# matsengrp/linearham

Hardware: AMD Instinct MI355X
Metric: phylo-HMM log-likelihood evals/sec (100-leaf x 400-site family) (higher is better)
Workload: dtype f64

## Files before the change

### linearham_amd/csrc/lh_forward.hip

```cpp
#include <cstdio>
#include <cstdlib>
#include <type_traits>

#include "lh_device.h"

namespace lh {

constexpr int kFwdThreads = 256;
constexpr int kFwdWaves = kFwdThreads / 64;
constexpr int kJunctionWaves = 4;

thread_local char g_k2a_form[64] = "", g_k2b_form[32] = "", g_forward_form[160] = "";
thread_local int g_k2b_dj_samples = 0;
thread_local int g_k2b_dj_waves = 0;

__device__ static inline int block_max_int(int v, int* red, int phase) {
#pragma unroll
  for (int off = 32; off > 0; off >>= 1) v = max(v, __shfl_xor(v, off, 64));
  int* r = red + phase * kFwdWaves;
  if ((threadIdx.x & 63) == 0) r[threadIdx.x >> 6] = v;
  __syncthreads();
  return max(max(r[0], r[1]), max(r[2], r[3]));
}

// ... 473 lines not shown
      lem[j] = l;
    }
  }
  if constexpr (kExt) {
    const int W1 = fam.vd.n_rows, W2 = fam.has_d ? fam.dj.n_rows : 0, NP = fam.n_prune;
    int32_t* jrs = jrs_all + s * (size_t)(W1 + W2);
    for (int r = tid; r < W1 + W2; r += kFwdThreads) {
      const int pat = r < W1 ? fam.vd.row_pat[r] : fam.dj.row_pat[r - W1];
      int smin = 0;
      if (kFromSiteLik && pat < NP) {
        smin = 0x7fffffff;
        for (int q = 0; q < R; ++q) smin = min(smin, site_scal[(s * R + q) * NP + pat]);
      }
      jrs[r] = smin;
    }
  }

  const int nV = fam.vgerm.n_genes, nD = fam.dgerm.n_genes, nJ = fam.jgerm.n_genes;
  double* gem = gem_all + s * fam.gem_size;
  const bool direct = *em_bad != 0;
  auto fill = [&](const DevSegments& seg, double* out, int phase) {
    if constexpr (kExt) return fill_segments_ext<kG, kByteOff>(seg, em, ems, tid, out, redi, phase);
    if (seg.cons_sites > 0 && !direct)
      return fill_consensus<kG, kByteOff>(seg, em, tid, out, redi, phase, cons_inv, cons_pv, cons_pk, cons_cap);
    return fill_segments<kG, kByteOff>(seg, em, tid, out, redi, phase);
  };
  int cv = fill(fam.vpadding, gem, 0);
  cv += fill(fam.vgerm, gem + nV, 1);
  int cd = 0, cj;
  if (small_sets_by_wave(fam, kExt, direct)) {
    const int wave = tid >> 6, lane = tid & 63;
    double* jg = gem + 2 * (size_t)nV + (fam.has_d ? nD : 0);
    int m = 0;
    if (wave == 1 && fam.has_d) m = fill_segments_wave<kByteOff>(fam.dgerm, em, lane, gem + 2 * (size_t)nV);
    if (wave == 2) m = fill_segments_wave<kByteOff>(fam.jgerm, em, lane, jg);
    if (wave == 3) m = fill_segments_wave<kByteOff>(fam.jpadding, em, lane, jg + nJ);
    if (lane == 0) redi[wave] = m;
    __syncthreads();
    cd = redi[1];
    cj = redi[2] + redi[3];
  } else if (fam.has_d) {
    cd = fill(fam.dgerm, gem + 2 * (size_t)nV, 0);
    cj = fill(fam.jgerm, gem + 2 * (size_t)nV + nD, 1);
    cj += fill(fam.jpadding, gem + 2 * (size_t)nV + nD + nJ, 0);
  } else {
    cj = fill(fam.jgerm, gem + 2 * (size_t)nV, 0);
    cj += fill(fam.jpadding, gem + 2 * (size_t)nV + nJ, 1);
  }
  if (tid == 0) {
    gcnt_all[s * 3 + 0] = cv;
    gcnt_all[s * 3 + 1] = cd;
    gcnt_all[s * 3 + 2] = cj;
  }
}


template <int kCtrl>
__device__ static inline double dpp_move(double v) {
  const int lo = __builtin_amdgcn_update_dpp(0, __double2loint(v), kCtrl, 0xf, 0xf, true);
  const int hi = __builtin_amdgcn_update_dpp(0, __double2hiint(v), kCtrl, 0xf, 0xf, true);
  return __hiloint2double(hi, lo);
}

__device__ static inline double read_lane(double v, int lane) {
  return __hiloint2double(__builtin_amdgcn_readlane(__double2hiint(v), lane),
                          __builtin_amdgcn_readlane(__double2loint(v), lane));
}

constexpr int kDppQuadSwap1 = 0xB1;
constexpr int kDppQuadSwap2 = 0x4E;
constexpr int kDppHalfMirror = 0x141;
constexpr int kDppMirror = 0x140;

__device__ static inline double wave_sum(double v) {
  v += dpp_move<kDppQuadSwap1>(v);
  v += dpp_move<kDppQuadSwap2>(v);
  v += dpp_move<kDppHalfMirror>(v);
  v += dpp_move<kDppMirror>(v);
  return (read_lane(v, 0) + read_lane(v, 16)) + (read_lane(v, 32) + read_lane(v, 48));
}

__device__ static inline unsigned scale_key(double v) { return (unsigned)__double2hiint(v) - 1u; }

template <int kCtrl>
__device__ static inline unsigned dpp_min_u32(unsigned v) {
  return min(v, (unsigned)__builtin_amdgcn_update_dpp(0, (int)v, kCtrl, 0xf, 0xf, true));
}

__device__ static inline unsigned wave_min_key(unsigned v) {
  v = dpp_min_u32<kDppQuadSwap1>(v);
  v = dpp_min_u32<kDppQuadSwap2>(v);
  v = dpp_min_u32<kDppHalfMirror>(v);
  v = dpp_min_u32<kDppMirror>(v);
  const unsigned a = __builtin_amdgcn_readlane((int)v, 0), b = __builtin_amdgcn_readlane((int)v, 16);
  const unsigned c = __builtin_amdgcn_readlane((int)v, 32), d = __builtin_amdgcn_readlane((int)v, 48);
  return min(min(a, b), min(c, d));
}

template <int kCtrl>
__device__ static inline unsigned dpp_max_u32(unsigned v) {
  return max(v, (unsigned)__builtin_amdgcn_update_dpp(0, (int)v, kCtrl, 0xf, 0xf, true));
}

__device__ static inline unsigned wave_max_u32(unsigned v) {
  v = dpp_max_u32<kDppQuadSwap1>(v);
  v = dpp_max_u32<kDppQuadSwap2>(v);
  v = dpp_max_u32<kDppHalfMirror>(v);
  v = dpp_max_u32<kDppMirror>(v);
  const unsigned a = __builtin_amdgcn_readlane((int)v, 0), b = __builtin_amdgcn_readlane((int)v, 16);
  const unsigned c = __builtin_amdgcn_readlane((int)v, 32), d = __builtin_amdgcn_readlane((int)v, 48);
  return max(max(a, b), max(c, d));
}

template <bool kExt>
__device__ static inline unsigned key_start() {
  return kExt ? 0u : 0xffffffffu;
}
template <bool kExt>
__device__ static inline unsigned key_add(unsigned key, double v) {
  return kExt ? max(key, (unsigned)__double2hiint(v)) : min(key, scale_key(v));
}

struct RowScale {
  int k;
  double factor;
  bool extra;
  __device__ double apply(double v) const {
    v *= factor;
    if (extra) v *= kScaleFactor;
    return v;
  }
};

__device__ static inline RowScale row_scale(unsigned min_key) {
  const unsigned hw = min_key + 1u;
  const unsigned e = (hw >> 20) & 0x7ffu;
  RowScale s;
  s.extra = hw != 0 && e == 0 && (hw & 0xfffffu) < (1u << 18);
  const int k3 = hw == 0 ? 0 : (e < 767u) + (e < 511u) + (e < 255u);
  s.k = k3 + (s.extra ? 1 : 0);
  s.factor = __hiloint2double((1023 + 256 * k3) << 20, 0);
  return s;
}

template <bool kExt>
__device__ static inline RowScale wave_row_scale(unsigned key) {
  return row_scale(kExt ? wave_max_u32(key) - 1u : wave_min_key(key));
}

__device__ static __forceinline__ RowScale pick(bool hi, const RowScale& sa, const RowScale& sb) {
  return RowScale{hi ? sb.k : sa.k, hi ? sb.factor : sa.factor, hi ? sb.extra : sa.extra};
}

struct RightRow {
  double nlo[4], rtr, rli;
  int ridx;
  int4 nx;
};

template <int GL, int GR>
struct RowTables {
  double ltr[GL], llo[GL];
  int lidx[GL];
  RightRow right[GR];
};

__device__ static __forceinline__ void load_right_row(const DevJunction& J, int i, unsigned r, RightRow& t) {
  const size_t orr = (size_t)i * J.right_pad;
  const double2* pn = reinterpret_cast<const double2*>(J.right_nlo) + 2 * orr;
  const double2 a = pn[2u * r], b = pn[2u * r + 1u];
  t.nlo[0] = a.x;
  t.nlo[1] = a.y;
  t.nlo[2] = b.x;
  t.nlo[3] = b.y;
  t.nx = (reinterpret_cast<const int4*>(J.nti_xmsa) + orr)[r];
  t.rtr = (J.right_trans + orr)[r];
  t.rli = (J.right_gp_li + orr)[r];
  t.ridx = (J.right_xmsa + orr)[r];
}

template <int GL, int GR>
__device__ static inline void load_row(const DevJunction& J, int i, unsigned lane, RowTables<GL, GR>& t) {
  const size_t ol = (size_t)i * J.left_pad;
  const double* lt = J.left_trans + ol;
  const double* ll = J.left_lo + ol;
  const int32_t* lx = J.left_xmsa + ol;
#pragma unroll
  for (int q = 0; q < GL; ++q) {
    t.ltr[q] = lt[lane + 64u * q];
    t.llo[q] = ll[lane + 64u * q];
    t.lidx[q] = lx[lane + 64u * q];
  }
#pragma unroll
  for (int q = 0; q < GR; ++q) load_right_row(J, i, lane + 64u * q, t.right[q]);
}


__device__ static __forceinline__ void load_nli(const DevJunction& J, unsigned r, double (&nli)[4]) {
  const double2* p = reinterpret_cast<const double2*>(J.right_gp_nli) + 2u * r;
  const double2 a = p[0], b = p[1];
  nli[0] = a.x, nli[1] = a.y, nli[2] = b.x, nli[3] = b.y;
}

template <bool kExt>
__device__ static __forceinline__ unsigned right_gene_step(unsigned key, double (&fN)[4], double& fR, double A,
                                                           const double (&nli)[4], const double* ntt_lds, unsigned r,
                                                           const RightRow& t, const double* jem) {
  const double n0 = fN[0], n1 = fN[1], n2 = fN[2], n3 = fN[3];
  const double2* tt = reinterpret_cast<const double2*>(ntt_lds) + 8u * r;
  const int nxs[4] = {t.nx.x, t.nx.y, t.nx.z, t.nx.w};
#pragma unroll
  for (int b = 0; b < 4; ++b) {
    const double2 t01 = tt[2 * b], t23 = tt[2 * b + 1];
    double s = ((n0 * t01.x + n1 * t01.y) + n2 * t23.x) + n3 * t23.y;
    s += A * nli[b];
    fN[b] = s * jem[nxs[b]];
  }
  double s = ((n0 * t.nlo[0] + n1 * t.nlo[1]) + n2 * t.nlo[2]) + n3 * t.nlo[3];
  s += fR * t.rtr;
  s += A * t.rli;
  fR = s * jem[t.ridx];
#pragma unroll
  for (int b = 0; b < 4; ++b) key = key_add<kExt>(key, fN[b]);
  return key_add<kExt>(key, fR);
}

__device__ static __forceinline__ double exit_handoff(const DevJunction& J, unsigned r, int nR, const double (&fN)[4],
                                                      double fR, double A, const double* __restrict__ germ_em,
                                                      const double* __restrict__ pad_trans,
                                                      const double* __restrict__ pad_em) {
  const double2* xn = reinterpret_cast<const double2*>(J.exit_nlo) + 2u * r;
  const double2 x01 = xn[0], x23 = xn[1];
  double s = ((fN[0] * x01.x + fN[1] * x01.y) + fN[2] * x23.x) + fN[3] * x23.y;
  s += fR * J.exit_trans[r];
  s += A * J.exit_gp_li[r];
  double v = 0.0;
  if ((int)r < nR) {
    v = s * germ_em[r];
    if (pad_trans) v *= pad_trans[r];
    if (pad_em) v *= pad_em[r];
  }
  return v;
}

__device__ static __forceinline__ void store_right(double* __restrict__ o, int nL, int nR, unsigned r,
                                                   const double (&fN)[4], double fR) {
  if ((int)r < nR) {
    o[nL + 4 * (size_t)r + 0] = fN[0];
    o[nL + 4 * (size_t)r + 1] = fN[1];
    o[nL + 4 * (size_t)r + 2] = fN[2];
    o[nL + 4 * (size_t)r + 3] = fN[3];
    o[nL + 4 * (size_t)nR + r] = fR;
  }
}

__device__ static __forceinline__ size_t junction_fwd_size(const DevJunction& J) {
  return (size_t)J.n_rows * (J.n_left + 5 * (size_t)J.n_right);
}

template <int GL, int GR, bool kExt>
__device__ static int junction_wave(const DevJunction& J, const double* jem, const double* ntt_lds, int lane,
                                    const double (&f_in)[GL], int count_in, const double* __restrict__ germ_em,
                                    const double* __restrict__ pad_trans, const double* __restrict__ pad_em,
                                    double (&g_out)[GR], double* __restrict__ fwd_out,
                                    int32_t* __restrict__ scal_out, const int32_t* __restrict__ jrs) {
  const int W = J.n_rows, nL = J.n_left, nR = J.n_right;
  int count = count_in;
  double fL[GL], fN[GR][4], fR[GR];
  double nli[GR][4];
#pragma unroll
  for (int q = 0; q < GL; ++q) fL[q] = f_in[q];
#pragma unroll
  for (int q = 0; q < GR; ++q) {
    fR[q] = 0.0;
    fN[q][0] = fN[q][1] = fN[q][2] = fN[q][3] = 0.0;
    load_nli(J, lane + 64u * q, nli[q]);
  }
  const size_t row_stride = (size_t)nL + 5 * (size_t)nR;
  double A;
  {
    double part = 0.0;
#pragma unroll
    for (int q = 0; q < GL; ++q) part += f_in[q] * J.enter_lo[lane + 64u * q];
    A = wave_sum(part);
  }

  auto step = [&](int i, const RowTables<GL, GR>& t) __attribute__((always_inline)) {
    unsigned key = key_start<kExt>();
    double part = 0.0;
#pragma unroll
    for (int q = 0; q < GL; ++q) {
      const double v = (fL[q] * t.ltr[q]) * jem[t.lidx[q]];
      fL[q] = v;
      key = key_add<kExt>(key, v);
      part += v * t.llo[q];
    }
#pragma unroll
    for (int q = 0; q < GR; ++q)
      key = right_gene_step<kExt>(key, fN[q], fR[q], A, nli[q], ntt_lds, lane + 64u * q, t.right[q], jem);
    A = wave_sum(part);
    const RowScale sc = wave_row_scale<kExt>(key);
    if constexpr (kExt) count += jrs[i];
    if (sc.k != 0) {
      A = sc.apply(A);
#pragma unroll
      for (int q = 0; q < GL; ++q) fL[q] = sc.apply(fL[q]);
#pragma unroll
      for (int q = 0; q < GR; ++q) {
        fR[q] = sc.apply(fR[q]);
#pragma unroll
        for (int b = 0; b < 4; ++b) fN[q][b] = sc.apply(fN[q][b]);
      }
      count += sc.k;
    }
    if (fwd_out) {
      double* o = fwd_out + (size_t)i * row_stride;
#pragma unroll
      for (int q = 0; q < GL; ++q) {
        const int g = lane + 64 * q;
        if (g < nL) o[g] = fL[q];
      }
#pragma unroll
      for (int q = 0; q < GR; ++q) store_right(o, nL, nR, lane + 64u * q, fN[q], fR[q]);
    }
    if (scal_out && lane == 0) scal_out[i] = count;
  };

  for (int i = 0; i < W; ++i) {
    RowTables<GL, GR> t;
    load_row<GL, GR>(J, i, lane, t);
    step(i, t);
  }

  unsigned key = key_start<kExt>();
#pragma unroll
  for (int q = 0; q < GR; ++q) {
    const double v = exit_handoff(J, lane + 64u * q, nR, fN[q], fR[q], A, germ_em, pad_trans, pad_em);
    key = key_add<kExt>(key, v);
    g_out[q] = v;
  }
  const RowScale last = wave_row_scale<kExt>(key);
#pragma unroll
  for (int q = 0; q < GR; ++q) g_out[q] = last.apply(g_out[q]);
  return count + last.k;
}


struct HalfPair {
  double a, b;
};

__device__ static inline HalfPair half_sums(double v) {
  v += dpp_move<kDppQuadSwap1>(v);
  v += dpp_move<kDppQuadSwap2>(v);
  v += dpp_move<kDppHalfMirror>(v);
  v += dpp_move<kDppMirror>(v);
  return HalfPair{read_lane(v, 0) + read_lane(v, 16), read_lane(v, 32) + read_lane(v, 48)};
}

struct HalfKeys {
  unsigned a, b;
};

template <bool kExt>
__device__ static inline HalfKeys half_keys(unsigned v) {
  if (kExt) {
    v = dpp_max_u32<kDppQuadSwap1>(v);
    v = dpp_max_u32<kDppQuadSwap2>(v);
    v = dpp_max_u32<kDppHalfMirror>(v);
    v = dpp_max_u32<kDppMirror>(v);
  } else {
    v = dpp_min_u32<kDppQuadSwap1>(v);
    v = dpp_min_u32<kDppQuadSwap2>(v);
    v = dpp_min_u32<kDppHalfMirror>(v);
    v = dpp_min_u32<kDppMirror>(v);
  }
  const unsigned a = __builtin_amdgcn_readlane((int)v, 0), b = __builtin_amdgcn_readlane((int)v, 16);
  const unsigned c = __builtin_amdgcn_readlane((int)v, 32), d = __builtin_amdgcn_readlane((int)v, 48);
  return kExt ? HalfKeys{max(a, b) - 1u, max(c, d) - 1u} : HalfKeys{min(a, b), min(c, d)};
}

template <bool kExt>
__device__ static int junction_pair(const DevJunction& J, const double* jem, const double* ntt_lds, int lane, bool hi,
                                    double f_in, int count_in, const double* __restrict__ germ_em,
                                    const double* __restrict__ pad_trans, const double* __restrict__ pad_em,
                                    double& g_out, double* __restrict__ fwd_out, int32_t* __restrict__ scal_out,
                                    const int32_t* __restrict__ jrs, bool valid) {
  const int W = J.n_rows, nL = J.n_left, nR = J.n_right;
  const unsigned g = lane & 31;
  int count = count_in;
  double fL = f_in, fR = 0.0, fN[4] = {0.0, 0.0, 0.0, 0.0}, nli[4];
  load_nli(J, g, nli);
  const size_t row_stride = (size_t)nL + 5 * (size_t)nR;
  auto mine = [&](const HalfPair& p) { return hi ? p.b : p.a; };
  double A = mine(half_sums(f_in * J.enter_lo[g]));
  for (int i = 0; i < W; ++i) {
    const size_t ol = (size_t)i * J.left_pad;
    const double ltr = J.left_trans[ol + g], llo = J.left_lo[ol + g];
    const int lidx = J.left_xmsa[ol + g];
    RightRow t;
    load_right_row(J, i, g, t);

    unsigned key = key_start<kExt>();
    {
      const double v = (fL * ltr) * jem[lidx];
      fL = v;
      key = key_add<kExt>(key, v);
    }
    const double part = fL * llo;
    key = right_gene_step<kExt>(key, fN, fR, A, nli, ntt_lds, g, t, jem);
    A = mine(half_sums(part));
    const HalfKeys hk = half_keys<kExt>(key);
    const RowScale sa = row_scale(hk.a), sb = row_scale(hk.b);
    if constexpr (kExt) count += jrs[i];
    if ((sa.k | sb.k) != 0) {
      const RowScale sc = pick(hi, sa, sb);
      A = sc.apply(A);
      fL = sc.apply(fL);
      fR = sc.apply(fR);
#pragma unroll
      for (int b = 0; b < 4; ++b) fN[b] = sc.apply(fN[b]);
      count += sc.k;
    }
    if (fwd_out && valid) {
      double* o = fwd_out + (size_t)i * row_stride;
      if ((int)g < nL) o[g] = fL;
      store_right(o, nL, nR, g, fN, fR);
    }
    if (scal_out && valid && g == 0) scal_out[i] = count;
  }
  g_out = exit_handoff(J, g, nR, fN, fR, A, germ_em, pad_trans, pad_em);
  const HalfKeys hk = half_keys<kExt>(key_add<kExt>(key_start<kExt>(), g_out));
  const RowScale last = pick(hi, row_scale(hk.a), row_scale(hk.b));
  g_out = last.apply(g_out);
  return count + last.k;
}

template <int GL, bool kExt>
__device__ static void junction_vd_pair(const DevJunction& J, const double* jemA, const double* jemB,
                                        const double* ntt_lds, int lane, bool hi, const double (&fA_in)[GL],
                                        const double (&fB_in)[GL], int countA_in, int countB_in,
                                        const double* __restrict__ germ_em_mine, double& g_out, int& count_mine,
                                        double* __restrict__ fwdA, double* __restrict__ fwdB,
                                        int32_t* __restrict__ scoA, int32_t* __restrict__ scoB,
                                        const int32_t* __restrict__ jrsA, const int32_t* __restrict__ jrsB) {
  const int W = J.n_rows, nL = J.n_left, nR = J.n_right;
  const unsigned g = lane & 31;
  const double* jemM = hi ? jemB : jemA;
  int countA = countA_in, countB = countB_in;
  double fA[GL], fB[GL], fN[4] = {0.0, 0.0, 0.0, 0.0}, fR = 0.0, nli[4];
#pragma unroll
  for (int q = 0; q < GL; ++q) {
    fA[q] = fA_in[q];
    fB[q] = fB_in[q];
  }
  load_nli(J, g, nli);
  const size_t row_stride = (size_t)nL + 5 * (size_t)nR;
  double AA, AB;
  {
    double pa = 0.0, pb = 0.0;
#pragma unroll
    for (int q = 0; q < GL; ++q) {
      const double lo = J.enter_lo[lane + 64u * q];
      pa += fA_in[q] * lo;
      pb += fB_in[q] * lo;
    }
    AA = wave_sum(pa);
    AB = wave_sum(pb);
  }
  auto combine = [](unsigned a, unsigned b) { return kExt ? max(a, b) : min(a, b); };
  for (int i = 0; i < W; ++i) {
    const size_t ol = (size_t)i * J.left_pad;
    unsigned keyA = key_start<kExt>(), keyB = key_start<kExt>();
    double partA = 0.0, partB = 0.0;
    {
      const double* lt = J.left_trans + ol;
      const double* ll = J.left_lo + ol;
      const int32_t* lx = J.left_xmsa + ol;
#pragma unroll
      for (int q = 0; q < GL; ++q) {
        const double ltr = lt[lane + 64u * q], llo = ll[lane + 64u * q];
        const int lidx = lx[lane + 64u * q];
        const double va = (fA[q] * ltr) * jemA[lidx];
        const double vb = (fB[q] * ltr) * jemB[lidx];
        fA[q] = va;
        fB[q] = vb;
        keyA = key_add<kExt>(keyA, va);
        keyB = key_add<kExt>(keyB, vb);
        partA += va * llo;
        partB += vb * llo;
      }
    }
    {
      RightRow t;
      load_right_row(J, i, g, t);
      const unsigned keyR = right_gene_step<kExt>(key_start<kExt>(), fN, fR, hi ? AB : AA, nli, ntt_lds, g, t, jemM);
      if (hi)
        keyB = combine(keyB, keyR);
      else
        keyA = combine(keyA, keyR);
    }
    AA = wave_sum(partA);
    AB = wave_sum(partB);
    const RowScale sa = wave_row_scale<kExt>(keyA), sb = wave_row_scale<kExt>(keyB);
    if constexpr (kExt) {
      countA += jrsA[i];
      countB += jrsB[i];
    }
    if ((sa.k | sb.k) != 0) {
      AA = sa.apply(AA);
      AB = sb.apply(AB);
#pragma unroll
      for (int q = 0; q < GL; ++q) {
        fA[q] = sa.apply(fA[q]);
        fB[q] = sb.apply(fB[q]);
      }
      const RowScale sm = pick(hi, sa, sb);
      fR = sm.apply(fR);
#pragma unroll
      for (int b = 0; b < 4; ++b) fN[b] = sm.apply(fN[b]);
      countA += sa.k;
      countB += sb.k;
    }
    if (fwdA) {
      double* oa = fwdA + (size_t)i * row_stride;
      double* ob = fwdB ? fwdB + (size_t)i * row_stride : nullptr;
#pragma unroll
      for (int q = 0; q < GL; ++q) {
        const int t = lane + 64 * q;
        if (t < nL) {
          oa[t] = fA[q];
          if (ob) ob[t] = fB[q];
        }
      }
      double* om = hi ? ob : oa;
      if (om) store_right(om, nL, nR, g, fN, fR);
    }
    if (lane == 0) {
      if (scoA) scoA[i] = countA;
      if (scoB) scoB[i] = countB;
    }
  }
  g_out = exit_handoff(J, g, nR, fN, fR, hi ? AB : AA, germ_em_mine, nullptr, nullptr);
  const HalfKeys hk = half_keys<kExt>(key_add<kExt>(key_start<kExt>(), g_out));
  const RowScale last = pick(hi, row_scale(hk.a), row_scale(hk.b));
  g_out = last.apply(g_out);
  count_mine = (hi ? countB : countA) + last.k;
}


__device__ static __forceinline__ void stage_ntt(double* dst, const double* __restrict__ src, int count, int threads) {
  for (int t = threadIdx.x; t < count; t += threads) dst[t] = src[t];
}

template <int kSamples>
__device__ static __forceinline__ void stage_jem(double* jem0, const double* __restrict__ jem_all, int first, int n,
                                                 int NJ, int lane) {
  for (int h = 0; h < kSamples; ++h) {
    const double* src = jem_all + (size_t)min(first + h, n - 1) * NJ;
    double* dst = jem0 + (size_t)h * (NJ + 1);
    for (int j = lane; j < NJ; j += 64) dst[j] = src[j];
    if (lane == 0) dst[NJ] = 0.0;
  }
  __builtin_amdgcn_fence(__ATOMIC_RELEASE, "wavefront");
  __builtin_amdgcn_wave_barrier();
  __builtin_amdgcn_fence(__ATOMIC_ACQUIRE, "wavefront");
}

template <int GA, bool kExt>
__device__ static __forceinline__ int initial_v_forward(const DevFamily& fam, const double* __restrict__ gem, int lane,
                                                        int cv, double (&gV)[GA], double* __restrict__ fwd,
                                                        int32_t* __restrict__ sco) {
  const int nV = fam.vgerm.n_genes;
  unsigned key = key_start<kExt>();
#pragma unroll
  for (int q = 0; q < GA; ++q) {
    const int t = lane + 64 * q;
    double v = 0.0;
    if (t < nV) {
      v = fam.vgerm_gene_prob[t];
      v *= fam.vpadding_transition[t];
      v *= gem[t];
      v *= fam.vgerm_trans_prod[t];
      v *= gem[nV + t];
    }
    key = key_add<kExt>(key, v);
    gV[q] = v;
  }
  const RowScale sc = wave_row_scale<kExt>(key);
#pragma unroll
  for (int q = 0; q < GA; ++q) gV[q] = sc.apply(gV[q]);
  const int vcount = cv + sc.k;
  if (fwd) {
#pragma unroll
    for (int q = 0; q < GA; ++q)
      if (lane + 64 * q < nV) fwd[lane + 64 * q] = gV[q];
  }
  if (sco && lane == 0) sco[0] = vcount;
  return vcount;
}

template <int GA, bool kExt>
__global__ void __launch_bounds__(64 * kJunctionWaves)
    junction_vd_kernel(const DevFamily fam, int n, const double* __restrict__ gem_all,
                       const int32_t* __restrict__ gcnt_all, const double* __restrict__ jem_all,
                       const int32_t* __restrict__ jrs_all, double* __restrict__ fwd_all,
                       int32_t* __restrict__ scal_all, double* __restrict__ dxf, int32_t* __restrict__ dxc) {
  extern __shared__ double jlds[];
  const int lane = threadIdx.x & 63, wave = threadIdx.x >> 6;
  const int s = blockIdx.x * kJunctionWaves + wave;
  const int NJ = fam.n_jcols;
  double* ntt_vd = jlds;
  double* jem = ntt_vd + 16 * (size_t)fam.vd.right_pad + (size_t)wave * (NJ + 1);
  stage_ntt(ntt_vd, fam.vd.right_ntt, 16 * fam.vd.right_pad, 64 * kJunctionWaves);
  __syncthreads();
  if (s >= n) return;
  const int nV = fam.vgerm.n_genes, nD = fam.dgerm.n_genes;
  const size_t vd_fwd = junction_fwd_size(fam.vd);
  stage_jem<1>(jem, jem_all, s, n, NJ, lane);
  const double* gem = gem_all + (size_t)s * fam.gem_size;
  const int cv = gcnt_all[(size_t)s * 3 + 0], cd = gcnt_all[(size_t)s * 3 + 1];
  double* fwd = fwd_all ? fwd_all + (size_t)s * fam.forward_size : nullptr;
  int32_t* sco = scal_all ? scal_all + (size_t)s * fam.scaler_size : nullptr;
  double gV[GA];
  const int vcount = initial_v_forward<GA, kExt>(fam, gem, lane, cv, gV, fwd, sco);
  double gD[1];
  const int dcount =
      cd + junction_wave<GA, 1, kExt>(fam.vd, jem, ntt_vd, lane, gV, vcount, gem + 2 * (size_t)nV, nullptr, nullptr, gD,
                                      fwd ? fwd + nV : nullptr, sco ? sco + 1 : nullptr,
                                      kExt ? jrs_all + (size_t)s * (fam.vd.n_rows + fam.dj.n_rows) : nullptr);
  if (fwd && lane < nD) fwd[nV + vd_fwd + lane] = gD[0];
  if (sco && lane == 0) sco[1 + fam.vd.n_rows] = dcount;
  if (lane < 32) dxf[(size_t)s * 32 + lane] = gD[0];
  if (lane == 0) dxc[s] = dcount;
}

constexpr int kVdPairWaves = 4;
template <int GA, bool kExt>
__global__ void __launch_bounds__(64 * kVdPairWaves)
    junction_vd2_kernel(const DevFamily fam, int n, const double* __restrict__ gem_all,
                        const int32_t* __restrict__ gcnt_all, const double* __restrict__ jem_all,
                        const int32_t* __restrict__ jrs_all, double* __restrict__ fwd_all,
                        int32_t* __restrict__ scal_all, double* __restrict__ dxf, int32_t* __restrict__ dxc) {
  extern __shared__ double jlds[];
  const int lane = threadIdx.x & 63, wave = threadIdx.x >> 6;
  const int NJ = fam.n_jcols;
  double* ntt_vd = jlds;
  double* jem0 = ntt_vd + 16 * (size_t)fam.vd.right_pad + (size_t)(2 * wave) * (NJ + 1);
  stage_ntt(ntt_vd, fam.vd.right_ntt, 16 * fam.vd.right_pad, 64 * kVdPairWaves);
  __syncthreads();
  const int p = blockIdx.x * kVdPairWaves + wave;
  if (2 * p >= n) return;
  const bool hi = lane >= 32;
  const int sA = 2 * p, sB = min(2 * p + 1, n - 1);
  const bool validB = 2 * p + 1 < n;
  stage_jem<2>(jem0, jem_all, sA, n, NJ, lane);
  const int nV = fam.vgerm.n_genes, nD = fam.dgerm.n_genes;
  const size_t vd_fwd = junction_fwd_size(fam.vd);
  const double* gemA = gem_all + (size_t)sA * fam.gem_size;
  const double* gemB = gem_all + (size_t)sB * fam.gem_size;
  double* fwdA = fwd_all ? fwd_all + (size_t)sA * fam.forward_size : nullptr;
  double* fwdB = fwd_all && validB ? fwd_all + (size_t)sB * fam.forward_size : nullptr;
  int32_t* scoA = scal_all ? scal_all + (size_t)sA * fam.scaler_size : nullptr;
  int32_t* scoB = scal_all && validB ? scal_all + (size_t)sB * fam.scaler_size : nullptr;
  double gA[GA], gB[GA];
  unsigned keyA = key_start<kExt>(), keyB = key_start<kExt>();
#pragma unroll
  for (int q = 0; q < GA; ++q) {
    const int t = lane + 64 * q;
    double va = 0.0, vb = 0.0;
    if (t < nV) {
      const double c0 = fam.vgerm_gene_prob[t], c1 = fam.vpadding_transition[t], c2 = fam.vgerm_trans_prod[t];
      va = c0;
      va *= c1;
      va *= gemA[t];
      va *= c2;
      va *= gemA[nV + t];
      vb = c0;
      vb *= c1;
      vb *= gemB[t];
      vb *= c2;
      vb *= gemB[nV + t];
    }
    keyA = key_add<kExt>(keyA, va);
    keyB = key_add<kExt>(keyB, vb);
    gA[q] = va;
    gB[q] = vb;
  }
  int countA = gcnt_all[(size_t)sA * 3 + 0], countB = gcnt_all[(size_t)sB * 3 + 0];
  {
    const RowScale sa = wave_row_scale<kExt>(keyA), sb = wave_row_scale<kExt>(keyB);
#pragma unroll
    for (int q = 0; q < GA; ++q) {
      gA[q] = sa.apply(gA[q]);
      gB[q] = sb.apply(gB[q]);
    }
    countA += sa.k;
    countB += sb.k;
  }
  if (fwdA) {
#pragma unroll
    for (int q = 0; q < GA; ++q)
      if (lane + 64 * q < nV) {
        fwdA[lane + 64 * q] = gA[q];
        if (fwdB) fwdB[lane + 64 * q] = gB[q];
      }
  }
  if (lane == 0) {
    if (scoA) scoA[0] = countA;
    if (scoB) scoB[0] = countB;
  }
  const size_t jr = (size_t)fam.vd.n_rows + fam.dj.n_rows;
  double gD;
  int count_mine;
  junction_vd_pair<GA, kExt>(fam.vd, jem0, jem0 + (NJ + 1), ntt_vd, lane, hi, gA, gB, countA, countB,
                             (hi ? gemB : gemA) + 2 * (size_t)nV, gD, count_mine, fwdA ? fwdA + nV : nullptr,
                             fwdB ? fwdB + nV : nullptr, scoA ? scoA + 1 : nullptr, scoB ? scoB + 1 : nullptr,
                             kExt ? jrs_all + (size_t)sA * jr : nullptr, kExt ? jrs_all + (size_t)sB * jr : nullptr);
  const unsigned g = lane & 31;
  const int dcount = gcnt_all[(size_t)(hi ? sB : sA) * 3 + 1] + count_mine;
  if (!hi || validB) {
    const int sM = hi ? sB : sA;
    double* fwdM = hi ? fwdB : fwdA;
    int32_t* scoM = hi ? scoB : scoA;
    if (fwdM && (int)g < nD) fwdM[nV + vd_fwd + g] = gD;
    if (scoM && g == 0) scoM[1 + fam.vd.n_rows] = dcount;
    dxf[(size_t)sM * 32 + g] = gD;
    if (g == 0) dxc[sM] = dcount;
  }
}

constexpr int kPairWaves = 4;

struct DjSample {
  const double *jgerm_em, *jpad_em;
  int cj;
  double* fwd;
  int32_t* sco;
  const int32_t* jrs;
};

template <bool kExt>
__device__ static __forceinline__ DjSample dj_sample(const DevFamily& fam, int s, const double* __restrict__ gem_all,
                                                     const int32_t* __restrict__ gcnt_all,
                                                     const int32_t* __restrict__ jrs_all, double* __restrict__ fwd_all,
                                                     int32_t* __restrict__ scal_all) {
  const int nV = fam.vgerm.n_genes, nD = fam.dgerm.n_genes, nJ = fam.jgerm.n_genes;
  DjSample d;
  d.jgerm_em = gem_all + (size_t)s * fam.gem_size + 2 * (size_t)nV + nD;
  d.jpad_em = d.jgerm_em + nJ;
  d.cj = gcnt_all[(size_t)s * 3 + 2];
  d.fwd = fwd_all ? fwd_all + (size_t)s * fam.forward_size + nV + junction_fwd_size(fam.vd) + nD : nullptr;
  d.sco = scal_all ? scal_all + (size_t)s * fam.scaler_size + 2 + fam.vd.n_rows : nullptr;
  d.jrs = kExt ? jrs_all + (size_t)s * (fam.vd.n_rows + fam.dj.n_rows) + fam.vd.n_rows : nullptr;
  return d;
}

template <class Total>
__device__ static __forceinline__ void dj_finish(const DevFamily& fam, const DjSample& d, int s, bool valid, unsigned g,
                                                 double gJ, int jcount, Total&& total, double* __restrict__ loglik) {
  if (d.fwd && valid && (int)g < fam.jgerm.n_genes) d.fwd[junction_fwd_size(fam.dj) + g] = gJ;
  if (d.sco && valid && g == 0) d.sco[fam.dj.n_rows] = jcount;
  const double part = total();
  if (valid && g == 0) loglik[s] = log(part) - jcount * kLogScaleFactor;
}

template <bool kExt>
__global__ void __launch_bounds__(64 * kPairWaves)
    junction_dj_kernel(const DevFamily fam, int n, const double* __restrict__ gem_all,
                       const int32_t* __restrict__ gcnt_all, const double* __restrict__ jem_all,
                       const int32_t* __restrict__ jrs_all, const double* __restrict__ dxf,
                       const int32_t* __restrict__ dxc, double* __restrict__ loglik, double* __restrict__ fwd_all,
                       int32_t* __restrict__ scal_all) {
  extern __shared__ double jlds[];
  const int lane = threadIdx.x & 63, wave = threadIdx.x >> 6;
  const int NJ = fam.n_jcols;
  double* ntt_dj = jlds;
  double* jem0 = ntt_dj + 16 * (size_t)fam.dj.right_pad + (size_t)(2 * wave) * (NJ + 1);
  stage_ntt(ntt_dj, fam.dj.right_ntt, 16 * fam.dj.right_pad, 64 * kPairWaves);
  __syncthreads();
  const int p = blockIdx.x * kPairWaves + wave;
  if (2 * p >= n) return;
  const bool hi = lane >= 32;
  const int s2 = 2 * p + (hi ? 1 : 0);
  const bool valid = s2 < n;
  const int sr = valid ? s2 : n - 1;
  stage_jem<2>(jem0, jem_all, 2 * p, n, NJ, lane);
  const unsigned g = lane & 31;
  const DjSample d = dj_sample<kExt>(fam, sr, gem_all, gcnt_all, jrs_all, fwd_all, scal_all);
  const double f_in = valid ? dxf[(size_t)s2 * 32 + g] : 0.0;
  const int dcount = valid ? dxc[s2] : 0;
  double gJ;
  const int jcount = d.cj + junction_pair<kExt>(fam.dj, jem0 + (size_t)(hi ? 1 : 0) * (NJ + 1), ntt_dj, lane, hi, f_in,
                                                dcount, d.jgerm_em, fam.jpadding_transition, d.jpad_em, gJ, d.fwd,
                                                d.sco, d.jrs, valid);
  dj_finish(fam, d, s2, valid, g, gJ, jcount, [&] {
    const HalfPair tot = half_sums(gJ);
    return hi ? tot.b : tot.a;
  }, loglik);
}

constexpr int kDppRowFirst = 0x150;

__device__ static inline double row_tree_sum(double v) {
  v += dpp_move<kDppQuadSwap1>(v);
  v += dpp_move<kDppQuadSwap2>(v);
  v += dpp_move<kDppHalfMirror>(v);
  v += dpp_move<kDppMirror>(v);
  return v;
}

template <int GL>
__device__ static inline double row_sums(const double (&p)[GL]) {
  double t = row_tree_sum(p[0]);
  if constexpr (GL == 2)
    t = t + row_tree_sum(p[1]);
  else
    t = t + 0.0;
  return dpp_move<kDppRowFirst>(t);
}

template <bool kExt>
__device__ static inline unsigned row_key(unsigned v) {
  if (kExt) {
    v = dpp_max_u32<kDppQuadSwap1>(v);
    v = dpp_max_u32<kDppQuadSwap2>(v);
    v = dpp_max_u32<kDppHalfMirror>(v);
    v = dpp_max_u32<kDppMirror>(v);
    return v - 1u;
  }
  v = dpp_min_u32<kDppQuadSwap1>(v);
  v = dpp_min_u32<kDppQuadSwap2>(v);
  v = dpp_min_u32<kDppHalfMirror>(v);
  v = dpp_min_u32<kDppMirror>(v);
  return v;
}

constexpr unsigned kRescaleKeyEnd = (767u << 20) - 1u;

template <int GL, bool kExt>
__device__ static int junction_quad(const DevJunction& J, const double* jem, const double* ntt_lds, unsigned l,
                                    const double (&f_in)[GL], int count_in, const double* __restrict__ germ_em,
                                    const double* __restrict__ pad_trans, const double* __restrict__ pad_em,
                                    double& g_out, double* __restrict__ fwd_out, int32_t* __restrict__ scal_out,
                                    const int32_t* __restrict__ jrs, bool valid) {
  const int W = J.n_rows, nL = J.n_left, nR = J.n_right;
  int count = count_in;
  double fL[GL], fR = 0.0, fN[4] = {0.0, 0.0, 0.0, 0.0}, nli[4];
#pragma unroll
  for (int q = 0; q < GL; ++q) fL[q] = f_in[q];
  load_nli(J, l, nli);
  const size_t row_stride = (size_t)nL + 5 * (size_t)nR;
  double A;
  {
    double part[GL];
#pragma unroll
    for (int q = 0; q < GL; ++q) part[q] = f_in[q] * J.enter_lo[l + 16u * q];
    A = row_sums<GL>(part);
  }
  for (int i = 0; i < W; ++i) {
    const size_t ol = (size_t)i * J.left_pad;
    double ltr[GL], llo[GL];
    int lidx[GL];
#pragma unroll
    for (int q = 0; q < GL; ++q) {
      ltr[q] = J.left_trans[ol + l + 16u * q];
      llo[q] = J.left_lo[ol + l + 16u * q];
      lidx[q] = J.left_xmsa[ol + l + 16u * q];
    }
    RightRow t;
    load_right_row(J, i, l, t);

    unsigned key = key_start<kExt>();
    double part[GL];
#pragma unroll
    for (int q = 0; q < GL; ++q) {
      const double v = (fL[q] * ltr[q]) * jem[lidx[q]];
      fL[q] = v;
      key = key_add<kExt>(key, v);
      part[q] = fL[q] * llo[q];
    }
// ... 119 lines not shown
    if (sco) sco += fam.dj.n_rows;
  } else {
    const double* jgerm_em = gem + 2 * (size_t)nV;
    const double* jpad_em = jgerm_em + nJ;
    jcount = cj + junction_wave<GA, GB, kExt>(fam.vd, jem, ntt_vd, lane, gV, vcount, jgerm_em,
                                              fam.jpadding_transition, jpad_em, gJ, fwd, sco, jrs);
    if (fwd) fwd += junction_fwd_size(fam.vd);
    if (sco) sco += fam.vd.n_rows;
  }
  if (fwd) {
#pragma unroll
    for (int q = 0; q < GB; ++q)
      if (lane + 64 * q < nJ) fwd[lane + 64 * q] = gJ[q];
  }
  if (sco && lane == 0) sco[0] = jcount;

  double part = 0.0;
#pragma unroll
  for (int q = 0; q < GB; ++q) part += gJ[q];
  part = wave_sum(part);
  if (lane == 0) loglik[s] = log(part) - jcount * kLogScaleFactor;
}

static size_t junction_lds_bytes(const DevFamily& fam) {
  return ((size_t)2 * kJunctionWaves * (fam.n_jcols + 1) +
          16 * ((size_t)fam.vd.right_pad + (fam.has_d ? fam.dj.right_pad : 0))) *
         sizeof(double);
}

static bool junction_pair_form(const DevFamily& fam) {
  static const bool off = debug_options().k2b_no_pair;
  return !off && fam.has_d && fam.dgerm.n_genes <= 32 && fam.jgerm.n_genes <= 32;
}

static size_t dj4_lds_bytes(const DevFamily& fam, int waves) {
  return ((size_t)4 * waves * (fam.n_jcols + 1) + 16 * 16) * sizeof(double);
}

static int dj4_waves(const DevFamily& fam, size_t lds_pair) {
  static const bool pair = debug_options().k2b_dj_pair;
  if (pair || fam.jgerm.n_genes > 16 || fam.dgerm.n_genes > 32) return 0;
  constexpr size_t kCuLds = 160 * 1024;
  auto per_simd = [](size_t lds, int waves) { return std::min<size_t>(4, lds > kCuLds ? 0 : kCuLds / lds * waves / 4); };
  const size_t need = per_simd(lds_pair, kPairWaves);
  for (int waves = 4; waves <= 16; waves *= 2)
    if (per_simd(dj4_lds_bytes(fam, waves), waves) >= need && need > 0) return waves;
  return 0;
}

static size_t emission_lds_bytes(const DevFamily& fam, bool ext) {
  const size_t cap = (size_t)cons_capacity(fam);
  return ((((size_t)fam.n_ucol + 2) & ~(size_t)1) + 6) * sizeof(double) + (2 * kFwdWaves + 2) * sizeof(int) +
         (cap ? (2 * cap + 4) * sizeof(double) + (cap + 4) * sizeof(int) : 0) +
         (ext ? ((size_t)fam.n_ucol + 2) * sizeof(int) : 0);
}

size_t forward_lds_bytes(const DevFamily& fam) {
  const size_t a = emission_lds_bytes(fam, true), b = junction_lds_bytes(fam);
  return a > b ? a : b;
}

template <class F>
static void with_bool(bool b, F&& f) {
  if (b)
    f(std::true_type{});
  else
    f(std::false_type{});
}
template <int N>
using slots_c = std::integral_constant<int, N>;

template <int kG, bool kSite, bool kByteOff, bool kExt, bool kLem>
static void launch_emission_l(const DevFamily& fam, const DevFamily* fam_dev, int n, int R, const double* site_lik,
                              const int32_t* site_scal, const double* pi, const double* em_in, double* em_out,
                              double* gem, int32_t* gcnt, double* jem, int32_t* jrs, const LogEmRequest& lem,
                              hipStream_t stream) {
  const size_t lds = emission_lds_bytes(fam, kExt);
  snprintf(g_k2a_form, sizeof(g_k2a_form), "emission<%d,%s,%s%s%s>", kG, kSite ? "site" : "caller",
           kByteOff ? "byte" : "index", kExt ? ",ext" : "", kLem ? ",lem" : "");
  launch_lds(emission_kernel<kG, kSite, kByteOff, kExt, kLem>, dim3(n), dim3(kFwdThreads), lds, stream, fam_dev, R,
             site_lik, site_scal, pi, em_in, em_out, gem, gcnt, jem, jrs, lem.cols, lem.n, lem.out);
}

template <int kG, bool kSite, bool kByteOff, bool kExt>
static void launch_emission_k(const DevFamily& fam, const DevFamily* fam_dev, int n, int R, const double* site_lik,
                              const int32_t* site_scal, const double* pi, const double* em_in, double* em_out,
                              double* gem, int32_t* gcnt, double* jem, int32_t* jrs, const LogEmRequest& lem,
                              hipStream_t stream) {
  if constexpr (kSite) {
    if (lem.out) {
      launch_emission_l<kG, kSite, kByteOff, kExt, true>(fam, fam_dev, n, R, site_lik, site_scal, pi, em_in, em_out, gem,
                                                         gcnt, jem, jrs, lem, stream);
      return;
    }
  }
  launch_emission_l<kG, kSite, kByteOff, kExt, false>(fam, fam_dev, n, R, site_lik, site_scal, pi, em_in, em_out, gem, gcnt,
                                                      jem, jrs, lem, stream);
}

template <int kG>
static void launch_emission_g(const DevFamily& fam, const DevFamily* fam_dev, int n, int R, const double* site_lik,
                              const int32_t* site_scal, const double* pi, const double* em_in, double* em_out,
                              double* gem, int32_t* gcnt, double* jem, int32_t* jrs, bool ext, const LogEmRequest& lem,
                              hipStream_t stream) {
  with_bool(site_lik != nullptr, [&](auto S) {
    with_bool(fam.idx_byte_offsets != 0, [&](auto B) {
      with_bool(ext, [&](auto E) {
        launch_emission_k<kG, decltype(S)::value, decltype(B)::value, decltype(E)::value>(
            fam, fam_dev, n, R, site_lik, site_scal, pi, em_in, em_out, gem, gcnt, jem, jrs, lem, stream);
      });
    });
  });
}

template <bool kExt>
static void launch_dj(const DevFamily& fam, int n, const double* gem, const int32_t* gcnt, const double* jem,
                      const int32_t* jrs, const double* dxf, const int32_t* dxc, double* loglik, double* forward_out,
                      int32_t* scaler_out, hipStream_t stream) {
  const size_t lds_dj = ((size_t)2 * kPairWaves * (fam.n_jcols + 1) + 16 * (size_t)fam.dj.right_pad) * sizeof(double);
  const int waves = dj4_waves(fam, lds_dj);
  g_k2b_dj_samples = waves == 0 ? 2 : 4;
  g_k2b_dj_waves = waves == 0 ? kPairWaves : waves;
  auto kernel = junction_dj_kernel<kExt>;
  size_t lds = lds_dj;
  dim3 grid(((n + 1) / 2 + kPairWaves - 1) / kPairWaves), block(64 * kPairWaves);
  if (waves != 0) {
    kernel = fam.dgerm.n_genes <= 16 ? junction_dj4_kernel<1, kExt> : junction_dj4_kernel<2, kExt>;
    lds = dj4_lds_bytes(fam, waves);
    grid = dim3(((n + 3) / 4 + waves - 1) / waves);
    block = dim3(64 * waves);
  }
  launch_lds(kernel, grid, block, lds, stream, fam, n, gem, gcnt, jem, jrs, dxf, dxc, loglik, forward_out, scaler_out);
}

template <int GA, int GB>
static void launch_junction_g(const DevFamily& fam, int n, const double* gem, const int32_t* gcnt, const double* jem,
                              const int32_t* jrs, double* dxf, int32_t* dxc, double* loglik, double* forward_out,
                              int32_t* scaler_out, bool ext, hipStream_t stream) {
  g_k2b_dj_samples = g_k2b_dj_waves = 0;
  if constexpr (GB == 1) {
    if (junction_pair_form(fam)) {
      const size_t jem_slice = (size_t)fam.n_jcols + 1, ntt_vd = 16 * (size_t)fam.vd.right_pad;
      bool vd2 = false;
      if constexpr (GA <= 4) {
        static const bool vd_single = debug_options().k2b_vd_single;
        vd2 = !vd_single;
      }
      snprintf(g_k2b_form, sizeof(g_k2b_form), vd2 ? "vd2<%d>+dj" : "vd<%d>+dj", GA);
      with_bool(ext, [&](auto E) {
        constexpr bool kE = decltype(E)::value;
        if constexpr (GA <= 4) {
          if (vd2)
            launch_lds(junction_vd2_kernel<GA, kE>, dim3(((n + 1) / 2 + kVdPairWaves - 1) / kVdPairWaves),
                       dim3(64 * kVdPairWaves), (2 * kVdPairWaves * jem_slice + ntt_vd) * sizeof(double), stream, fam, n,
                       gem, gcnt, jem, jrs, forward_out, scaler_out, dxf, dxc);
        }
        if (!vd2)
          launch_lds(junction_vd_kernel<GA, kE>, dim3((n + kJunctionWaves - 1) / kJunctionWaves),
                     dim3(64 * kJunctionWaves), (kJunctionWaves * jem_slice + ntt_vd) * sizeof(double), stream, fam, n,
                     gem, gcnt, jem, jrs, forward_out, scaler_out, dxf, dxc);
        launch_dj<kE>(fam, n, gem, gcnt, jem, jrs, dxf, dxc, loglik, forward_out, scaler_out, stream);
      });
      return;
    }
  }
  snprintf(g_k2b_form, sizeof(g_k2b_form), "junction<%d,%d>", GA, GB);
  with_bool(ext, [&](auto E) {
    launch_lds(junction_kernel<GA, GB, decltype(E)::value>, dim3((n + kJunctionWaves - 1) / kJunctionWaves),
               dim3(64 * kJunctionWaves), junction_lds_bytes(fam), stream, fam, n, gem, gcnt, jem, jrs, loglik,
               forward_out, scaler_out);
  });
}

template <int GA>
static void launch_junction_a(int gb, const DevFamily& fam, int n, const double* gem, const int32_t* gcnt,
                              const double* jem, const int32_t* jrs, double* dxf, int32_t* dxc, double* loglik,
                              double* forward_out, int32_t* scaler_out, bool ext, hipStream_t stream) {
  if (gb <= 1)
    launch_junction_g<GA, 1>(fam, n, gem, gcnt, jem, jrs, dxf, dxc, loglik, forward_out, scaler_out, ext, stream);
  else if (gb <= 2)
    launch_junction_g<GA, 2>(fam, n, gem, gcnt, jem, jrs, dxf, dxc, loglik, forward_out, scaler_out, ext, stream);
  else
    launch_junction_g<GA, 4>(fam, n, gem, gcnt, jem, jrs, dxf, dxc, loglik, forward_out, scaler_out, ext, stream);
}

void launch_forward(const DevFamily& fam, const DevFamily* fam_dev, int n, int R, const double* site_lik,
                    const int32_t* site_scal, const double* pi, const double* em_in, double* em_out, double* gem,
                    int32_t* gcnt, double* jem, int32_t* jrs, double* dxf, int32_t* dxc, double* loglik,
                    double* forward_out, int32_t* scaler_out, bool ext, hipStream_t stream, const LogEmRequest& lem) {
  const int slots = (fam.max_genes + kFwdThreads - 1) / kFwdThreads;
  auto emission = [&](auto G) {
    launch_emission_g<decltype(G)::value>(fam, fam_dev, n, R, site_lik, site_scal, pi, em_in, em_out, gem, gcnt, jem, jrs,
                                          ext, lem, stream);
  };
  if (slots <= 1)
    emission(slots_c<1>{});
  else if (slots <= 2)
    emission(slots_c<2>{});
  else
    emission(slots_c<4>{});
  const int ga = (fam.vgerm.n_genes + 63) / 64;
  const int gb = (std::max(fam.dgerm.n_genes, fam.jgerm.n_genes) + 63) / 64;
  auto junction = [&](auto G) {
    launch_junction_a<decltype(G)::value>(gb, fam, n, gem, gcnt, jem, jrs, dxf, dxc, loglik, forward_out, scaler_out, ext,
                                          stream);
  };
  if (ga <= 1)
    junction(slots_c<1>{});
  else if (ga <= 2)
    junction(slots_c<2>{});
  else if (ga <= 4)
    junction(slots_c<4>{});
  else if (ga <= 8)
    junction(slots_c<8>{});
  else
    junction(slots_c<16>{});
  const int cons = ext ? 0
                       : (fam.vpadding.cons_sites > 0) | (fam.vgerm.cons_sites > 0) << 1 | (fam.dgerm.cons_sites > 0) << 2 |
                             (fam.jgerm.cons_sites > 0) << 3 | (fam.jpadding.cons_sites > 0) << 4;
  snprintf(g_forward_form, sizeof(g_forward_form), "%s cons=%d small=%s | %s", g_k2a_form, cons,
           small_sets_by_wave(fam, ext, false) ? "wave" : "block", g_k2b_form);
}

const char* forward_last_form() { return g_forward_form; }
int forward_last_dj_samples() { return g_k2b_dj_samples; }
int forward_last_dj_waves() { return g_k2b_dj_waves; }

}
```

Before: 8.744 million.

## Cut register pressure in VD pair junction kernel via scalar bases and LDS relayout

Reworks the VD pair junction loop to reduce VGPR/SGPR pressure. It forces row bases into scalar registers with precomputed lane byte offsets, re-reads kernel arguments from the kernarg segment after the main loop instead of keeping them live, and folds the two half-row scale reductions into one permlane32 swap plus a single DPP reduction. It also stages the NTT table entry-major in LDS so lanes read contiguous entries. The trade-off is heavy reliance on inline-asm register constraints and a hardcoded 32-gene staging size, which assumes right_pad equals 32.

```diff
diff --git a/linearham_amd/csrc/lh_forward.hip b/linearham_amd/csrc/lh_forward.hip
--- a/linearham_amd/csrc/lh_forward.hip
+++ b/linearham_amd/csrc/lh_forward.hip
@@ -649,6 +649,36 @@
   return RowScale{hi ? sb.k : sa.k, hi ? sb.factor : sa.factor, hi ? sb.extra : sa.extra};
 }
 
+template <class T>
+using global_ptr = T __attribute__((address_space(1)))*;
+__device__ static __forceinline__ int scalar_again(int i) {
+  asm("; lh: row %0" : "+s"(i));
+  return i;
+}
+__device__ static __forceinline__ uint64_t row_base(const void* p) {
+  uint64_t v = reinterpret_cast<uint64_t>(p);
+  asm("; lh: row table at %0" : "+s"(v));
+  return v;
+}
+struct LaneOffsets {
+  unsigned b4, b8, b16, b32;
+  __device__ explicit LaneOffsets(unsigned e) : b4(4u * e), b8(8u * e), b16(16u * e), b32(32u * e) {}
+};
+template <class... U>
+__device__ static __forceinline__ void offsets_again(U&... o) {
+  auto one = [](unsigned& v) { asm("; lh: lane offset %0" : "+v"(v)); };
+  (one(o), ...);
+}
+template <class T>
+__device__ static __forceinline__ T row_load(uint64_t base, unsigned lane_off, unsigned more = 0) {
+  return *(global_ptr<const T>)(base + lane_off + more);
+}
+template <class T>
+__device__ static __forceinline__ void row_store(uint64_t base, unsigned lane_off, unsigned more, T v) {
+  asm volatile("; lh: lane offset %0" : "+v"(lane_off));
+  *(global_ptr<T>)(base + lane_off + more) = v;
+}
+
 struct RightRow {
   double nlo[4], rtr, rli;
   int ridx;
@@ -676,6 +706,23 @@
   t.ridx = (J.right_xmsa + orr)[r];
 }
 
+typedef double vec2d __attribute__((ext_vector_type(2)));
+typedef int vec4i __attribute__((ext_vector_type(4)));
+__device__ static __forceinline__ void load_right_row_at(const DevJunction& J, int i, const LaneOffsets& r, RightRow& t) {
+  const size_t orr = (size_t)i * J.right_pad;
+  const uint64_t pn = row_base(J.right_nlo + 4 * orr);
+  const vec2d a = row_load<vec2d>(pn, r.b32), b = row_load<vec2d>(pn, r.b32, 16);
+  t.nlo[0] = a.x;
+  t.nlo[1] = a.y;
+  t.nlo[2] = b.x;
+  t.nlo[3] = b.y;
+  const vec4i nx = row_load<vec4i>(row_base(J.nti_xmsa + 4 * orr), r.b16);
+  t.nx = make_int4(nx.x, nx.y, nx.z, nx.w);
+  t.rtr = row_load<double>(row_base(J.right_trans + orr), r.b8);
+  t.rli = row_load<double>(row_base(J.right_gp_li + orr), r.b8);
+  t.ridx = row_load<int>(row_base(J.right_xmsa + orr), r.b4);
+}
+
 template <int GL, int GR>
 __device__ static inline void load_row(const DevJunction& J, int i, unsigned lane, RowTables<GL, GR>& t) {
   const size_t ol = (size_t)i * J.left_pad;
@@ -699,16 +746,17 @@
   nli[0] = a.x, nli[1] = a.y, nli[2] = b.x, nli[3] = b.y;
 }
 
-template <bool kExt>
+template <bool kExt, int kByEntry = 0>
 __device__ static __forceinline__ unsigned right_gene_step(unsigned key, double (&fN)[4], double& fR, double A,
                                                            const double (&nli)[4], const double* ntt_lds, unsigned r,
                                                            const RightRow& t, const double* jem) {
   const double n0 = fN[0], n1 = fN[1], n2 = fN[2], n3 = fN[3];
-  const double2* tt = reinterpret_cast<const double2*>(ntt_lds) + 8u * r;
+  constexpr unsigned kPair = kByEntry ? kByEntry : 1;
+  const double2* tt = reinterpret_cast<const double2*>(ntt_lds) + (kByEntry ? r : 8u * r);
   const int nxs[4] = {t.nx.x, t.nx.y, t.nx.z, t.nx.w};
 #pragma unroll
   for (int b = 0; b < 4; ++b) {
-    const double2 t01 = tt[2 * b], t23 = tt[2 * b + 1];
+    const double2 t01 = tt[2 * b * kPair], t23 = tt[(2 * b + 1) * kPair];
     double s = ((n0 * t01.x + n1 * t01.y) + n2 * t23.x) + n3 * t23.y;
     s += A * nli[b];
     fN[b] = s * jem[nxs[b]];
@@ -875,6 +923,12 @@
   const unsigned a = __builtin_amdgcn_readlane((int)v, 0), b = __builtin_amdgcn_readlane((int)v, 16);
   const unsigned c = __builtin_amdgcn_readlane((int)v, 32), d = __builtin_amdgcn_readlane((int)v, 48);
   return kExt ? HalfKeys{max(a, b) - 1u, max(c, d) - 1u} : HalfKeys{min(a, b), min(c, d)};
+}
+
+template <class Op>
+__device__ static __forceinline__ unsigned fold_halves(unsigned a, unsigned b, Op op) {
+  const auto s = __builtin_amdgcn_permlane32_swap(a, b, false, false);
+  return op(s[0], s[1]);
 }
 
 template <bool kExt>
@@ -933,8 +987,16 @@
   return count + last.k;
 }
 
-template <int GL, bool kExt>
-__device__ static void junction_vd_pair(const DevJunction& J, const double* jemA, const double* jemB,
+template <class T>
+__device__ static __forceinline__ const T& kernel_args_again() {
+  uint64_t v = reinterpret_cast<uint64_t>(__builtin_amdgcn_kernarg_segment_ptr());
+  asm volatile("; lh: kernel arguments at %0, read again from here" : "+s"(v));
+  return *(const T*)(const T __attribute__((address_space(4)))*)v;
+}
+
+template <int GL, bool kExt, class ExitJunction>
+__device__ static void junction_vd_pair(const DevJunction& J, ExitJunction exit_junction, const double* jemA,
+                                        const double* jemB,
                                         const double* ntt_lds, int lane, bool hi, const double (&fA_in)[GL],
                                         const double (&fB_in)[GL], int countA_in, int countB_in,
                                         const double* __restrict__ germ_em_mine, double& g_out, int& count_mine,
@@ -966,18 +1028,20 @@
     AB = wave_sum(pb);
   }
   auto combine = [](unsigned a, unsigned b) { return kExt ? max(a, b) : min(a, b); };
-  for (int i = 0; i < W; ++i) {
+  LaneOffsets offL(lane), offR(g);
+  unsigned g_row = g;
+  for (int row = 0; row < W; ++row) {
+    const int i = scalar_again(row);
+    offsets_again(offL.b4, offL.b8, offR.b4, offR.b8, offR.b16, offR.b32, g_row);
     const size_t ol = (size_t)i * J.left_pad;
     unsigned keyA = key_start<kExt>(), keyB = key_start<kExt>();
     double partA = 0.0, partB = 0.0;
     {
-      const double* lt = J.left_trans + ol;
-      const double* ll = J.left_lo + ol;
-      const int32_t* lx = J.left_xmsa + ol;
+      const uint64_t lt = row_base(J.left_trans + ol), ll = row_base(J.left_lo + ol), lx = row_base(J.left_xmsa + ol);
 #pragma unroll
       for (int q = 0; q < GL; ++q) {
-        const double ltr = lt[lane + 64u * q], llo = ll[lane + 64u * q];
-        const int lidx = lx[lane + 64u * q];
+        const double ltr = row_load<double>(lt, offL.b8, 512u * q), llo = row_load<double>(ll, offL.b8, 512u * q);
+        const int lidx = row_load<int>(lx, offL.b4, 256u * q);
         const double va = (fA[q] * ltr) * jemA[lidx];
         const double vb = (fB[q] * ltr) * jemB[lidx];
         fA[q] = va;
@@ -988,18 +1052,16 @@
         partB += vb * llo;
       }
     }
+    unsigned keyR;
     {
       RightRow t;
-      load_right_row(J, i, g, t);
-      const unsigned keyR = right_gene_step<kExt>(key_start<kExt>(), fN, fR, hi ? AB : AA, nli, ntt_lds, g, t, jemM);
-      if (hi)
-        keyB = combine(keyB, keyR);
-      else
-        keyA = combine(keyA, keyR);
+      load_right_row_at(J, i, offR, t);
+      keyR = right_gene_step<kExt, 32>(key_start<kExt>(), fN, fR, hi ? AB : AA, nli, ntt_lds, g_row, t, jemM);
     }
     AA = wave_sum(partA);
     AB = wave_sum(partB);
-    const RowScale sa = wave_row_scale<kExt>(keyA), sb = wave_row_scale<kExt>(keyB);
+    const HalfKeys hk = half_keys<kExt>(combine(fold_halves(keyA, keyB, combine), keyR));
+    const RowScale sa = row_scale(hk.a), sb = row_scale(hk.b);
     if constexpr (kExt) {
       countA += jrsA[i];
       countB += jrsB[i];
@@ -1020,25 +1082,31 @@
       countB += sb.k;
     }
     if (fwdA) {
-      double* oa = fwdA + (size_t)i * row_stride;
-      double* ob = fwdB ? fwdB + (size_t)i * row_stride : nullptr;
-#pragma unroll
-      for (int q = 0; q < GL; ++q) {
-        const int t = lane + 64 * q;
-        if (t < nL) {
-          oa[t] = fA[q];
-          if (ob) ob[t] = fB[q];
+      int nLr = nL;
+      asm volatile("; lh: left genes %0" : "+s"(nLr));
+      auto store_row = [&](double* o, const double (&fM)[GL], bool right) {
+        const uint64_t left = row_base(o), nti = row_base(o + nLr), germ = row_base(o + nLr + 4 * (size_t)nR);
+#pragma unroll
+        for (int q = 0; q < GL; ++q)
+          if ((int)(lane + 64u * q) < nLr) row_store(left, offL.b8, 512u * q, fM[q]);
+        if (right && (int)g < nR) {
+#pragma unroll
+          for (int b = 0; b < 4; ++b) row_store(nti, offR.b32, 8u * b, fN[b]);
+          row_store(germ, offR.b8, 0, fR);
         }
+      };
+      store_row(fwdA + (size_t)i * row_stride, fA, !hi);
+      if (fwdB) store_row(fwdB + (size_t)i * row_stride, fB, hi);
+    }
+    if (scoA) {
+      if (lane == 0) scoA[i] = countA;
+      if (scoB) {
+        if (lane == 0) scoB[i] = countB;
       }
-      double* om = hi ? ob : oa;
-      if (om) store_right(om, nL, nR, g, fN, fR);
-    }
-    if (lane == 0) {
-      if (scoA) scoA[i] = countA;
-      if (scoB) scoB[i] = countB;
-    }
-  }
-  g_out = exit_handoff(J, g, nR, fN, fR, hi ? AB : AA, germ_em_mine, nullptr, nullptr);
+    }
+  }
+  const DevJunction& Jx = exit_junction();
+  g_out = exit_handoff(Jx, g, Jx.n_right, fN, fR, hi ? AB : AA, germ_em_mine, nullptr, nullptr);
   const HalfKeys hk = half_keys<kExt>(key_add<kExt>(key_start<kExt>(), g_out));
   const RowScale last = pick(hi, row_scale(hk.a), row_scale(hk.b));
   g_out = last.apply(g_out);
@@ -1048,6 +1116,14 @@
 
 __device__ static __forceinline__ void stage_ntt(double* dst, const double* __restrict__ src, int count, int threads) {
   for (int t = threadIdx.x; t < count; t += threads) dst[t] = src[t];
+}
+
+template <int kGenes>
+__device__ static __forceinline__ void stage_ntt_by_entry(double* dst, const double* __restrict__ src, int threads) {
+  for (int t = threadIdx.x; t < 16 * kGenes; t += threads) {
+    const int r = t >> 4, e = (t >> 1) & 7;
+    dst[2 * (e * kGenes + r) + (t & 1)] = src[t];
+  }
 }
 
 template <int kSamples>
@@ -1133,18 +1209,34 @@
 }
 
 constexpr int kVdPairWaves = 4;
+struct Vd2Args {
+  DevFamily fam;
+  int n;
+  const double* gem_all;
+  const int32_t* gcnt_all;
+  const double* jem_all;
+  const int32_t* jrs_all;
+  double* fwd_all;
+  int32_t* scal_all;
+  double* dxf;
+  int32_t* dxc;
+};
 template <int GA, bool kExt>
-__global__ void __launch_bounds__(64 * kVdPairWaves)
-    junction_vd2_kernel(const DevFamily fam, int n, const double* __restrict__ gem_all,
-                        const int32_t* __restrict__ gcnt_all, const double* __restrict__ jem_all,
-                        const int32_t* __restrict__ jrs_all, double* __restrict__ fwd_all,
-                        int32_t* __restrict__ scal_all, double* __restrict__ dxf, int32_t* __restrict__ dxc) {
+__global__ void __launch_bounds__(64 * kVdPairWaves) junction_vd2_kernel(const Vd2Args args) {
+  const DevFamily& fam = args.fam;
+  const int n = args.n;
+  const double* __restrict__ gem_all = args.gem_all;
+  const int32_t* __restrict__ gcnt_all = args.gcnt_all;
+  const double* __restrict__ jem_all = args.jem_all;
+  const int32_t* __restrict__ jrs_all = args.jrs_all;
+  double* __restrict__ fwd_all = args.fwd_all;
+  int32_t* __restrict__ scal_all = args.scal_all;
   extern __shared__ double jlds[];
-  const int lane = threadIdx.x & 63, wave = threadIdx.x >> 6;
+  const int lane = threadIdx.x & 63, wave = __builtin_amdgcn_readfirstlane(threadIdx.x >> 6);
   const int NJ = fam.n_jcols;
   double* ntt_vd = jlds;
   double* jem0 = ntt_vd + 16 * (size_t)fam.vd.right_pad + (size_t)(2 * wave) * (NJ + 1);
-  stage_ntt(ntt_vd, fam.vd.right_ntt, 16 * fam.vd.right_pad, 64 * kVdPairWaves);
+  stage_ntt_by_entry<32>(ntt_vd, fam.vd.right_ntt, 64 * kVdPairWaves);
   __syncthreads();
   const int p = blockIdx.x * kVdPairWaves + wave;
   if (2 * p >= n) return;
@@ -1152,8 +1244,7 @@
   const int sA = 2 * p, sB = min(2 * p + 1, n - 1);
   const bool validB = 2 * p + 1 < n;
   stage_jem<2>(jem0, jem_all, sA, n, NJ, lane);
-  const int nV = fam.vgerm.n_genes, nD = fam.dgerm.n_genes;
-  const size_t vd_fwd = junction_fwd_size(fam.vd);
+  const int nV = fam.vgerm.n_genes;
   const double* gemA = gem_all + (size_t)sA * fam.gem_size;
   const double* gemB = gem_all + (size_t)sB * fam.gem_size;
   double* fwdA = fwd_all ? fwd_all + (size_t)sA * fam.forward_size : nullptr;
@@ -1210,20 +1301,23 @@
   const size_t jr = (size_t)fam.vd.n_rows + fam.dj.n_rows;
   double gD;
   int count_mine;
-  junction_vd_pair<GA, kExt>(fam.vd, jem0, jem0 + (NJ + 1), ntt_vd, lane, hi, gA, gB, countA, countB,
-                             (hi ? gemB : gemA) + 2 * (size_t)nV, gD, count_mine, fwdA ? fwdA + nV : nullptr,
-                             fwdB ? fwdB + nV : nullptr, scoA ? scoA + 1 : nullptr, scoB ? scoB + 1 : nullptr,
-                             kExt ? jrs_all + (size_t)sA * jr : nullptr, kExt ? jrs_all + (size_t)sB * jr : nullptr);
+  junction_vd_pair<GA, kExt>(
+      fam.vd, []() -> const DevJunction& { return kernel_args_again<Vd2Args>().fam.vd; }, jem0, jem0 + (NJ + 1), ntt_vd,
+      lane, hi, gA, gB, countA, countB, (hi ? gemB : gemA) + 2 * (size_t)nV, gD, count_mine, fwdA ? fwdA + nV : nullptr,
+      fwdB ? fwdB + nV : nullptr, scoA ? scoA + 1 : nullptr, scoB ? scoB + 1 : nullptr,
+      kExt ? jrs_all + (size_t)sA * jr : nullptr, kExt ? jrs_all + (size_t)sB * jr : nullptr);
+  const Vd2Args& again = kernel_args_again<Vd2Args>();
+  const int nV2 = again.fam.vgerm.n_genes, nD2 = again.fam.dgerm.n_genes;
   const unsigned g = lane & 31;
-  const int dcount = gcnt_all[(size_t)(hi ? sB : sA) * 3 + 1] + count_mine;
+  const int dcount = again.gcnt_all[(size_t)(hi ? sB : sA) * 3 + 1] + count_mine;
   if (!hi || validB) {
     const int sM = hi ? sB : sA;
     double* fwdM = hi ? fwdB : fwdA;
     int32_t* scoM = hi ? scoB : scoA;
-    if (fwdM && (int)g < nD) fwdM[nV + vd_fwd + g] = gD;
-    if (scoM && g == 0) scoM[1 + fam.vd.n_rows] = dcount;
-    dxf[(size_t)sM * 32 + g] = gD;
-    if (g == 0) dxc[sM] = dcount;
+    if (fwdM && (int)g < nD2) fwdM[nV2 + junction_fwd_size(again.fam.vd) + g] = gD;
+    if (scoM && g == 0) scoM[1 + again.fam.vd.n_rows] = dcount;
+    again.dxf[(size_t)sM * 32 + g] = gD;
+    if (g == 0) again.dxc[sM] = dcount;
   }
 }
 
@@ -1649,8 +1743,8 @@
         if constexpr (GA <= 4) {
           if (vd2)
             launch_lds(junction_vd2_kernel<GA, kE>, dim3(((n + 1) / 2 + kVdPairWaves - 1) / kVdPairWaves),
-                       dim3(64 * kVdPairWaves), (2 * kVdPairWaves * jem_slice + ntt_vd) * sizeof(double), stream, fam, n,
-                       gem, gcnt, jem, jrs, forward_out, scaler_out, dxf, dxc);
+                       dim3(64 * kVdPairWaves), (2 * kVdPairWaves * jem_slice + ntt_vd) * sizeof(double), stream,
+                       Vd2Args{fam, n, gem, gcnt, jem, jrs, forward_out, scaler_out, dxf, dxc});
         }
         if (!vd2)
           launch_lds(junction_vd_kernel<GA, kE>, dim3((n + kJunctionWaves - 1) / kJunctionWaves),
```

After: 8.794 million, median of 6. About the same (+0.6%).
